# yl602019618/Reconstruction-of-PDE-without-Time-Label

Measured on AMD Instinct MI355X. Metric: snapshot-bags/sec (train step) + rel-L2 drift error, 2D FPE 128² @1/2/4/8 GPU, higher is better.
Workload: dtype f32; 1 GPU; 2d_FPE train_fno.py NIOFP2D_FNO(2,3,100,25,3,12,32,2) (C), grid 128x128; per_gpu_batch=4, global_batch=4, T=100, bag_size=L=randint(50,T) with replacement, dataset_bags=4096, parallelism=dp1, optimizer=Adam lr 0.0005 (fused flat), launch=hip-graph per bag size L (all kernels replayed each step)

## Files before the change

include/blindno.h:

```cpp
#ifndef BLINDNO_H
#define BLINDNO_H

#include <stdint.h>

#ifdef __cplusplus
extern "C" {
#endif

typedef void* blindno_stream_t;

int blindno_abi_version(void);
const char* blindno_error_string(int code);


int blindno_lift_fwd(const float* in, const float* w0, const float* b0, float* x0,
                     int Bn, int N1, int N2, int Cin, int C, int P1, int P2,
                     blindno_stream_t stream);

int blindno_lift_bwd(const float* dx0, const float* in, const float* w0, float* d_in,
                     float* partial, int nchunk,
                     int Bn, int N1, int N2, int Cin, int C, int P1, int P2,
                     blindno_stream_t stream);
int blindno_lift_bwd_nchunk(int Bn, int N1, int N2);

// ... 212 lines not shown
                        int width, blindno_stream_t stream);
int blindno_bagattn_bwd(const float* grid, const float* u, const float* dy, const float* w,
                        const float* A, const float* cs, float* partial, float* dm, float* M,
                        float* du, float* dgt, int B, int L, int S, int width,
                        blindno_stream_t stream);


int blindno_mse(const float* p, const float* t, float* partial, float* grad, int64_t n,
                int nblk, const float* gscale, blindno_stream_t stream);
int blindno_mse_finish(const float* partial, int nblk, int64_t n, float* loss,
                       blindno_stream_t stream);
int blindno_mse_finish_acc(const float* partial, int nblk, int64_t n, float* loss, float* acc,
                           blindno_stream_t stream);
int blindno_mse_fwd(const float* p, const float* t, float* partial, int64_t n, int nblk,
                    float* loss, float* acc, unsigned* counter, float* grad,
                    blindno_stream_t stream);

int blindno_rowsq(const float* a, const float* b, double* out, int rows, int n, int stride,
                  int off_a, int off_b, int den_all, blindno_stream_t stream);

int blindno_gather_flat(const void* const* srcs, const int64_t* offs, const int64_t* ns, int nseg,
                        float* dst, blindno_stream_t stream);
int blindno_gather_batch(const void* const* srcs, void* const* dsts, const int64_t* rows,
                         const int64_t* nsrc, int nseg, const int64_t* ids, int B,
                         blindno_stream_t stream);
int blindno_adam(float* p, const float* g, float* m, float* v, int64_t n, double beta1,
                 double beta2, float eps, float step_size, float bc2s, float gscale,
                 blindno_stream_t stream);


int blindno_gpe_solve(const double* psi0, const double* V, const double* g, const double* kappa,
                      double dx, double dt, int nsteps, int order, int rec_every, double* rec_abs,
                      double* rec_psi, double* psi_out, int B, int Nx, int psi0_batched,
                      blindno_stream_t stream);

int blindno_trapz_rows(const double* a, const double* b, const double* x, double* out, int rows,
                       int n, blindno_stream_t stream);

int blindno_fp_propagate(const double* p0, const double* coef, double* out, int B, int nx,
                         int ny, int nout, int substeps, int degree, double dt_out,
                         blindno_stream_t stream);

int blindno_lift_fwd_g(const float* in, const float* w0, const float* b0, float* x0, int G,
                       int64_t wgs, int Bn, int N1, int N2, int Cin, int C, int P1, int P2,
                       blindno_stream_t stream);
int blindno_lift_bwd_g(const float* dx0, const float* in, const float* w0, float* d_in,
                       float* partial, int nchunk, int G, int64_t wgs, int Bn, int N1, int N2,
                       int Cin, int C, int P1, int P2, blindno_stream_t stream);
int blindno_lift_bag_ok(int G, int Bn, int N1, int N2, int Cin, int C, int P1, int P2);
int blindno_lift_fwd_bag_g(const float* in, const float* w0, const float* b0, float* x0, int G,
                           int64_t wgs, int Bn, int N1, int N2, int Cin, int C, int P1, int P2,
                           const float* ubar, const float* grid, const float* bw, const float* bb,
                           float invL, blindno_stream_t stream);
int blindno_lift_bwd_bag_mix_g(const float* dx0, const float* in, const float* w0, float* d_in,
                               float* partial, int nchunk, int G, int64_t wgs, int Bn, int N1,
                               int N2, int Cin, int C, int P1, int P2, const float* Xs,
                               const float* Gs, float* dWt, float* mpartial, int mnsplit, int K1,
                               int m2, const float* ubar, const float* grid, const float* bw,
                               const float* bb, float invL, float invLb, blindno_stream_t stream);
int blindno_lift_bwd_mix_g(const float* dx0, const float* in, const float* w0, float* d_in,
                           float* partial, int nchunk, int G, int64_t wgs, int Bn, int N1, int N2,
                           int Cin, int C, int P1, int P2, const float* Xs, const float* Gs,
                           float* dWt, float* mpartial, int mnsplit, int K1, int m2,
                           blindno_stream_t stream);
int blindno_project_fwd_g(const float* z, const float* w1, const float* b1, const float* w2,
                          const float* b2, float* out, int G, int64_t wgs, int Bn, int C, int P1,
                          int P2, int Ho, int Wo, int Hd, int Cout, int ostride, int ooff,
                          blindno_stream_t stream);
int blindno_project_bwd_g(const float* z, const float* w1, const float* b1, const float* w2,
                          const float* dout, float* dz, float* partial, int nchunk, int G,
                          int64_t wgs, int Bn, int C, int P1, int P2, int Ho, int Wo, int Hd,
                          int Cout, int ostride, int ooff, blindno_stream_t stream);
int blindno_colpass_g(const float* At, const float* Wt, float* Xs, float* Y, float* Z,
                      const float* FB, const float* GB, int G, int64_t wtgs, int Bn, int Ci,
                      int Co, int P1, int m1, int m2, int P2, int dir, blindno_stream_t stream);
int blindno_mix_wgrad_g(const float* X, const float* Gs, float* dWt, float* partial, int nsplit,
                        int G, int Bn, int Ci, int Co, int K1, int m2, blindno_stream_t stream);
int blindno_rowidft_epi_g(const float* Z, const float* x, const float* wc, const float* bc,
                          float* z, const float* tb, int G, int64_t wgs, int Bn, int C, int P1,
                          int P2, int m2, int act, blindno_stream_t stream);
int blindno_rowidft_bwd_g(const float* Gs, const float* dz, const float* wc, const float* xsrc,
                          float* dx, const float* tb, int G, int64_t wgs, int Bn, int C, int P1,
                          int P2, int m2, int act, blindno_stream_t stream);
int blindno_conv_wgrad_g(const float* dz, const float* x, float* partial, int nchunk, int G,
                         int Bn, int C, int P1, int P2, int act, blindno_stream_t stream);
int blindno_rowdft_wgrad_ok(int Bn, int C, int P1, int P2, int m2);
int blindno_rowdft_wgrad_g(const float* dz, const float* src, float* At, const float* Tp,
                           float* cpartial, int cnchunk, int act, const float* Xs,
                           const float* Gs, float* dWt, float* mpartial, int mnsplit, int K1,
                           int G, int Bn, int C, int P1, int P2, int m2, blindno_stream_t stream);

int blindno_bn_act_nslices(int N, int C, int HW);
int blindno_bn_act_fwd(const float* z, const float* gamma, const float* beta, float* run_mean,
                       float* run_var, float* y, float* save, float* partial, int N, int Npad,
                       int C, int HW, float eps, float momentum, float slope, int training,
                       blindno_stream_t stream);
int blindno_bn_act_bwd(const float* dy, const float* z, const float* gamma, const float* save,
                       float* dz, float* dgamma, float* dbeta, float* partial, float* coef, int N,
                       int Npad, int C, int HW, float slope, int training, blindno_stream_t stream);

int blindno_conv2d_fwd(const float* x, const float* w, const float* b, float* y, int N, int Ci,
                       int Hi, int Wi, int Co, int KH, int KW, int sh, int sw, int ph, int pw,
                       blindno_stream_t stream);
int blindno_conv2d_bwd_data(const float* dy, const float* w, float* dx, int N, int Ci, int Hi,
                            int Wi, int Co, int KH, int KW, int sh, int sw, int ph, int pw,
                            blindno_stream_t stream);
int blindno_conv2d_wgrad_nsplit(int N, int Ci, int Hi, int Wi, int Co, int KH, int KW, int sh,
                                int sw, int ph, int pw);
int blindno_conv2d_bwd_weight(const float* dy, const float* x, float* dwb, float* partial,
                              int nsplit, int N, int Ci, int Hi, int Wi, int Co, int KH, int KW,
                              int sh, int sw, int ph, int pw, blindno_stream_t stream);
int blindno_conv2d_fwd_nsplit(int N, int Ci, int Hi, int Wi, int Co, int KH, int KW, int sh,
                              int sw, int ph, int pw);
int blindno_conv2d_bwd_data_nsplit(int N, int Ci, int Hi, int Wi, int Co, int KH, int KW, int sh,
                                   int sw, int ph, int pw);
int blindno_conv2d_wscratch_floats(int mode, int N, int Ci, int Hi, int Wi, int Co, int KH, int KW,
                                   int sh, int sw, int ph, int pw);
int blindno_conv2d_fwd_split(const float* x, const float* w, const float* b, float* y,
                             float* partial, int nsplit, float* wscratch, int N, int Ci, int Hi,
                             int Wi, int Co, int KH, int KW, int sh, int sw, int ph, int pw,
                             blindno_stream_t stream);
int blindno_conv2d_bwd_data_split(const float* dy, const float* w, float* dx, float* partial,
                                  int nsplit, float* wscratch, int N, int Ci, int Hi, int Wi,
                                  int Co, int KH, int KW, int sh, int sw, int ph, int pw,
                                  blindno_stream_t stream);

int64_t blindno_spectral2d_tables_bytes(int P1, int P2, int m1, int m2);
int blindno_spectral2d_tables_init(void* tables, int P1, int P2, int m1, int m2);
int64_t blindno_spectral_conv2d_workspace_bytes(int Bn, int Ci, int Co, int P1, int P2, int m1,
                                                int m2, int bwd);
int64_t blindno_spectral_conv2d_saved_bytes(int Bn, int Ci, int P1, int m1, int m2);
int blindno_spectral_conv2d_fwd(const float* x, const float* w1, const float* w2, float* y,
                                float* saved, void* work, const void* tables, int Bn, int Ci,
                                int Co, int P1, int P2, int m1, int m2, blindno_stream_t stream);
int blindno_spectral_conv2d_bwd(const float* dy, const float* saved, const float* w1,
                                const float* w2, float* dx, float* dw1, float* dw2, void* work,
                                const void* tables, int Bn, int Ci, int Co, int P1, int P2,
                                int m1, int m2, blindno_stream_t stream);
int64_t blindno_spectral1d_tables_bytes(int P2, int m);
int blindno_spectral1d_tables_init(void* tables, int P2, int m);
int64_t blindno_spectral_conv1d_workspace_bytes(int Bn, int Ci, int Co, int P2, int m, int bwd);
int64_t blindno_spectral_conv1d_saved_bytes(int Bn, int Ci, int m);
int blindno_spectral_conv1d_fwd(const float* x, const float* w, float* y, float* saved,
                                void* work, const void* tables, int Bn, int Ci, int Co, int P2,
                                int m, blindno_stream_t stream);
int blindno_spectral_conv1d_bwd(const float* dy, const float* saved, const float* w, float* dx,
                                float* dw, void* work, const void* tables, int Bn, int Ci,
                                int Co, int P2, int m, blindno_stream_t stream);

int blindno_dwconv_fwd(const float* x, const float* w, const float* b, float* y, int N, int C,
                       int H, int W, int KH, int KW, blindno_stream_t stream);
int blindno_dwconv_bwd_data(const float* dy, const float* w, float* dx, int N, int C, int H,
                            int W, int KH, int KW, blindno_stream_t stream);
int blindno_dwconv_wgrad_nsplit(int N, int C, int H, int W);
int blindno_dwconv_bwd_weight(const float* dy, const float* x, float* dwb, float* partial,
                              int nsplit, int N, int C, int H, int W, int KH, int KW,
                              blindno_stream_t stream);
int blindno_cnx_pw_fwd(const float* xd, const float* sc, const float* lw, const float* lb,
                       const float* w1, const float* b1, const float* w2, const float* b2, float* y,
                       int N, int C, int HW, blindno_stream_t stream);
int blindno_cnx_pw_bwd_nblk(int N, int C, int HW);
int blindno_cnx_pw_bwd(const float* dy, const float* xd, const float* lw, const float* lb,
                       const float* w1, const float* b1, const float* w2, float* dxd,
                       float* dparams, float* partial, int nblk, int N, int C, int HW,
                       blindno_stream_t stream);
int blindno_maxpool_fwd(const float* x, float* y, uint8_t* arg, int NC, int H, int W, int KH,
// ... 66 lines not shown
```

reconstruction-of-pde-without-time-label_amd/blindno/_lib.py:

```python
from __future__ import annotations

import ctypes
import os
import threading

import torch

_HERE = os.path.dirname(os.path.abspath(__file__))
LIB_PATH = os.environ.get("BLINDNO_LIB", os.path.join(_HERE, "libblindno.so"))

SIGNATURES = {
    "blindno_abi_version": "",
    "blindno_lift_fwd": "ppppiiiiiiis",
    "blindno_lift_bwd": "pppppiiiiiiiis",
    "blindno_project_fwd": "ppppppiiiiiiiiiis",
    "blindno_project_bwd": "pppppppiiiiiiiiiiiis",
    "blindno_rowdft": "pppiiiiiis",
    "blindno_rowdft_crop": "pppiiiiiiiis",
    "blindno_rowdft_bag_lift": "ppppppiiiiiiiiis",
    "blindno_rowdft_bag_lift_dg": "pppppppiiiiiiiiis",
    "blindno_rowidft_epi_lift": "ppppppppppiiiiiiiiis",
    "blindno_rowidft_bwd_lift": "ppppppppppiiiiiiiiis",
    "blindno_colpass": "pppppppiiiiiiiis",
    "blindno_colspec_ok": "iiiiii",
    "blindno_colspec_nchunk": "ii",
    "blindno_colspec_bwd_nchunk": "ii",
    "blindno_rowdft_cd": "ppppiiiiiiiis",
    "blindno_rowdft_bag_lift_cd": "pppppiiiiiiiis",
    "blindno_rowdft_bag_lift_cd_pack": "pppppiiiiiiiippppis",
    "blindno_colmix": "pipppiiiiiiiippps",
    "blindno_rowidft_epi_zc": "ppppppppp" + "iiiiiiiiii" + "s",
    "blindno_rowidft_epi_lift_zc": "ppppppppppppp" + "iiiiiiiiiii" + "s",
    "blindno_rowidft_bwd_zc": "pppppppppp" + "iiiiiiiii" + "s",
    "blindno_rowidft_bwd_lift_zc": "ppppppppppp" + "iiiiiiiiii" + "s",
    "blindno_rowidft_bwd_lift_zc_mix": "ppppppppppp" + "iiiiiiiiii" + "ppppi" + "s",
    "blindno_rowdft_cd_bag": "pppi" + "ppp" + "iiiiiii" + "s",
    "blindno_rowidft_bwd_zc_bag": "pppp" + "i" + "pppppppp" + "iiiiiiiii" + "s",
    "blindno_mix_wgrad": "ppppiiiiiis",
    "blindno_mix_wgrad_part": "pppiiiiiiis",
    "blindno_mix_wgrad_multi": "ppppis",
    "blindno_mix_wgrad_multi_u": "ppppppis",
    "blindno_mix1d": "ppppiiiiiis",
    "blindno_rowidft_epi": "ppppppiiiiiis",
    "blindno_rowidft_epi_crop": "pppppp" + "iiiiiiii" + "s",
    "blindno_rowidft_bwd": "pppppppiiiiiis",
    "blindno_rowidft_bwd_crop": "pppppppiiiiiiiis",
    "blindno_rowidft_bwd_rd": "pppppppiiiiiiiipps",
    "blindno_rowidft_epi_rd": "ppppppiiiiiippis",
    "blindno_rowidft_epi_lift_rd": "ppppppppppiiiiiiiiippis",
    "blindno_conv_wgrad": "pppiiiiiis",
    "blindno_reduce_partials": "ppiis",
    "blindno_spectrum_tile_layout": "iiiii",
    "blindno_pack_w2d": "pppiiiiis",
    "blindno_unpack_w2d": "pppiiiiis",
    "blindno_pack_w1d": "ppiiiis",
    "blindno_bagmean_fwd": "pppppiiiiis",
    "blindno_bagmean_bwd": "pppiiiiis",
    "blindno_mse": "pppplips",
    "blindno_mse_finish": "pilps",
    "blindno_mse_finish_acc": "pilpps",
    "blindno_mse_fwd": "ppplipppps",
    "blindno_rowsq": "pppiiiiiis",
    "blindno_adam": "pppplddffffs",
    "blindno_gpe_solve": "ppppddiiipppiiis",
    "blindno_trapz_rows": "ppppiis",
    "blindno_lift_bwd_nchunk": "iii",
    "blindno_conv_wgrad_nchunk": "iii",
    "blindno_rowidft_bwd_nchunk": "iiiii",
    "blindno_set_rowfuse": "i",
    "blindno_set_colfuse": "i",
    "blindno_project_bwd_nchunk": "iii",
    "blindno_project_bwd_nchunk_heads": "iii",
    "blindno_mix_wgrad_nsplit": "iiiii",
    "blindno_lift_fwd_g": "ppppiliiiiiiis",
    "blindno_lift_fwd_bag_g": "ppppiliiiiiiippppfs",
    "blindno_lift_bag_ok": "iiiiiiii",
    "blindno_lift_bwd_g": "pppppiiliiiiiiis",
    "blindno_lift_bwd_mix_g": "pppppiiliiiiiiippppiiis",
    "blindno_lift_bwd_bag_mix_g": "pppppiiliiiiiiippppiiippppffs",
    "blindno_project_fwd_g": "ppppppiliiiiiiiiiis",
    "blindno_project_bwd_g": "pppppppiiliiiiiiiiiis",
    "blindno_colpass_g": "pppppppiliiiiiiiis",
    "blindno_mix_wgrad_g": "ppppiiiiiiis",
    "blindno_rowidft_epi_g": "ppppppiliiiiiis",
    "blindno_rowidft_bwd_g": "ppppppiliiiiiis",
    "blindno_conv_wgrad_g": "pppiiiiiiis",
    "blindno_rowdft_wgrad_ok": "iiiii",
    "blindno_rowdft_wgrad_g": "pppppiippppiiiiiiiis",
    "blindno_bagmean_fwd_w": "pppppp" + "iiiii" + "s",
    "blindno_project_bwd_w": "pppppppp" + "i" + "iiiiiiiiiii" + "s",
    "blindno_project_bag_stats_floats": "iii",
    "blindno_project_bag_bwd_nchunk": "iii",
    "blindno_project_bag_fwd": "ppppppppp" + "iiiiiiii" + "s",
    "blindno_project_bag_bwd": "ppppppp" + "i" + "iiiiiiii" + "s",
    "blindno_pack_w2d_2": "ppppp" + "iiiii" + "s",
    "blindno_unpack_w2d_2": "ppppp" + "iiiii" + "s",
    "blindno_bn_act_nslices": "iii",
    "blindno_bn_act_fwd": "ppppppppiiiifffis",
    "blindno_bn_act_bwd": "pppppppppiiiifis",
    "blindno_gather_flat": "pppips",
    "blindno_gather_batch": "ppppipis",
    "blindno_reduce_partials_multi": "ppppis",
    "blindno_reduce_partials_pieces": "ppppppis",
    "blindno_reduce_partials_pieces_u": "pppppppppis",
    "blindno_reduce_segs_limit": "i",
    "blindno_finish_multi": "pppppppppippppis",
    "blindno_unpack_w2d_multi": "ppppis",
    "blindno_pack_w2d_multi": "ppppis",
    "blindno_fp_propagate": "pppiiiiiids",
    "blindno_bagattn_nchunk": "i",
    "blindno_bagattn_fwd": "pppppppp" + "iiii" + "s",
    "blindno_bagattn_bwd": "ppppppppppp" + "iiii" + "s",
    "blindno_conv2d_fwd": "pppp" + "iiiiiiiiiii" + "s",
    "blindno_conv2d_bwd_data": "ppp" + "iiiiiiiiiii" + "s",
    "blindno_conv2d_wgrad_nsplit": "iiiiiiiiiii",
    "blindno_conv2d_bwd_weight": "pppp" + "i" + "iiiiiiiiiii" + "s",
    "blindno_conv2d_fwd_nsplit": "iiiiiiiiiii",
    "blindno_conv2d_fwd_split": "ppppp" + "i" + "p" + "iiiiiiiiiii" + "s",
    "blindno_conv2d_bwd_data_nsplit": "iiiiiiiiiii",
    "blindno_conv2d_bwd_data_split": "pppp" + "i" + "p" + "iiiiiiiiiii" + "s",
    "blindno_conv2d_wscratch_floats": "i" + "iiiiiiiiiii",
    "blindno_spectral2d_tables_bytes": "iiii",
    "blindno_spectral2d_tables_init": "piiii",
    "blindno_spectral_conv2d_workspace_bytes": "iiiiiiii",
    "blindno_spectral_conv2d_saved_bytes": "iiiii",
    "blindno_spectral_conv2d_fwd": "ppppppp" + "iiiiiii" + "s",
    "blindno_spectral_conv2d_bwd": "ppppppppp" + "iiiiiii" + "s",
    "blindno_spectral1d_tables_bytes": "ii",
    "blindno_spectral1d_tables_init": "pii",
    "blindno_spectral_conv1d_workspace_bytes": "iiiiii",
    "blindno_spectral_conv1d_saved_bytes": "iii",
    "blindno_spectral_conv1d_fwd": "pppppp" + "iiiii" + "s",
    "blindno_spectral_conv1d_bwd": "ppppppp" + "iiiii" + "s",
    "blindno_dwconv_fwd": "pppp" + "iiiiii" + "s",
    "blindno_dwconv_bwd_data": "ppp" + "iiiiii" + "s",
    "blindno_dwconv_wgrad_nsplit": "iiii",
    "blindno_dwconv_bwd_weight": "pppp" + "i" + "iiiiii" + "s",
    "blindno_cnx_pw_fwd": "ppppppppp" + "iii" + "s",
    "blindno_cnx_pw_bwd_nblk": "iii",
    "blindno_cnx_pw_bwd": "pppppppppp" + "iiii" + "s",
    "blindno_maxpool_fwd": "ppp" + "iiiii" + "s",
    "blindno_maxpool_bwd": "ppp" + "iiiii" + "s",
    "blindno_convt_fwd": "pppp" + "iiiiiiiii" + "s",
    "blindno_convt_bwd_data": "ppp" + "iiiiiiiii" + "s",
    "blindno_convt_wgrad_nparts": "iii",
    "blindno_convt_bwd_weight": "pppp" + "iiiiiiiii" + "s",
    "blindno_tok_gram_nchunk": "l",
    "blindno_tok_attn_save_floats": "iil",
    "blindno_tok_attn_fwd": "ppppppp" + "iil" + "f" + "s",
    "blindno_tok_attn_bwd_scratch_floats": "ii",
    "blindno_tok_attn_bwd": "pppppppp" + "iil" + "s",
    "blindno_deeponet_bag_nblk": "i",
    "blindno_deeponet_bag_fwd": "pppppp" + "iiii" + "f" + "s",
    "blindno_deeponet_bag_bwd": "pppppppp" + "iiiii" + "f" + "s",
    "blindno_spectral3d_ok": "iiiiiiiii",
    "blindno_colpass3d": "ppppppp" + "iiiiiiiiii" + "s",
    "blindno_pack_w3d": "ppppp" + "iiiiiiii" + "s",
    "blindno_unpack_w3d": "ppppp" + "iiiiiiii" + "s",
    "blindno_lift3d_fwd": "pppp" + "iiiiiiiii" + "s",
    "blindno_lift3d_bwd_nchunk": "iiii",
    "blindno_lift3d_bwd": "ppppp" + "i" + "iiiiiiiii" + "s",
    "blindno_project3d_fwd": "pppppp" + "iiiiiiiiii" + "s",
    "blindno_project3d_bwd_nchunk": "iiii",
    "blindno_project3d_bwd": "ppppppp" + "i" + "iiiiiiiiii" + "s",
}

SIGNATURES_CONV3D = {
    "blindno_conv3d_fwd_nsplit": "i" * 15,
# ... 120 lines not shown
```

reconstruction-of-pde-without-time-label_amd/blindno/ops.py:

```python
from __future__ import annotations

import contextlib
import ctypes
import math
from typing import List, Optional, Sequence, Tuple

import torch

from ._lib import BlindnoError, call, ptr, query, stream_ptr

F32 = torch.float32

MIX_F16 = False

BAG_STATS = True
BAG_STATS_MAX_BYTES = 4 << 30

COLSPEC = True
HEAD_BWD_MERGED = True
UNPACK_FOLD = True
HOST_ENC_MIX = True
HOST_PACK = True


# ... 1154 lines not shown
        offs.append(o)
        o += t.numel()
    return offs, o


def pack_heads_ahead(meta: FNOMeta, shape, prms, device):
    if not (GROUPED_HEADS and grouped_ok(meta, shape, prms)):
        return
    G, n = len(prms), meta.n_layers
    P1 = _fno_geometry(shape, meta)[4]
    K1 = kept_rows_count(meta.m1, P1)
    C = meta.width
    Wt_all = torch.empty(n, G, meta.m2, K1, C, C, 2, dtype=F32, device=device)
    segs = [(prms[g][2 + 4 * k], prms[g][3 + 4 * k]) for k in range(n) for g in range(G)]
    pack_ahead(segs, [Wt_all[k, g] for k in range(n) for g in range(G)], P1, Wt_all)


def grouped_ok(meta: FNOMeta, inp, prms) -> bool:
    if meta.dim != 2 or len(prms) != 2:
        return False
    n = meta.n_layers
    fc1w, fc2w = prms[0][2 + 4 * n], prms[0][4 + 4 * n]
    Hd, Cout = fc1w.shape[0], fc2w.shape[0]
    if Hd != 128 or meta.width > 15 or Cout > 2:
        return False
    if any(a.shape != b.shape for a, b in zip(prms[0], prms[1])):
        return False
    Bg, N1, N2, Cin, P1, P2, Ho, Wo = _fno_geometry(inp, meta)
    return (Bg * Ho * Wo) % 64 == 0 and P1 % 4 == 0


def _sub(buf, off):
    return buf[off:] if off else buf


class _GroupWeights:

    def __init__(self, smalls):
        d = None
        direct = all(t.is_contiguous() and t.dtype == F32 for sm in smalls for t in sm)
        for g in range(1, len(smalls)):
            for a, b in zip(smalls[0], smalls[g]):
                diff = b.data_ptr() - a.data_ptr()
                if diff % (4 * g) or (d is not None and diff != g * d):
                    direct = False
                    break
                d = diff // g
        if direct and d:
            self.base, self.buf, self.S = list(smalls[0]), None, d // 4
        else:
            self.offs, self.S = _offsets(smalls[0])
            self.buf = torch.cat([t.reshape(-1) for sm in smalls for t in sm])
            self.base = None

    def p(self, i):
        return ptr(self.base[i]) if self.base is not None else ptr(_sub(self.buf, self.offs[i]))


def fno_forward_grouped(meta: FNOMeta, inp, prms, bag=None):
    G = len(prms)
    Bg, N1, N2, Cin, P1, P2, Ho, Wo = _fno_geometry(inp if bag is None else bag.shape(inp), meta)
    Bn = G * Bg
    C, n = meta.width, meta.n_layers
    smalls = [_small_params(p, n, 2) for p in prms]
    small = _GroupWeights(smalls)
    S = small.S
    x0 = _empty(Bn, C, P1, P2, like=inp)
    if bag is None:
        call("blindno_lift_fwd_g", ptr(inp), small.p(0), small.p(1), ptr(x0),
             G, S, Bn, N1, N2, Cin, C, P1, P2, stream_ptr())
    else:
        call("blindno_lift_fwd_bag_g", None, small.p(0), small.p(1), ptr(x0), G, S, Bn, N1, N2, Cin, C,
             P1, P2, ptr(inp), ptr(bag.grid), ptr(bag.w), ptr(bag.b), 1.0, stream_ptr())
    K1 = kept_rows_count(meta.m1, P1)
    K1p = 16 * ((K1 + 15) // 16)
    FB, GB = twiddle_cols(P1, meta.m1, inp.device)
    src, act = x0, 0
    Xs, Wts, zs = [], [], []
    segs = [(prms[g][2 + 4 * k], prms[g][3 + 4 * k]) for k in range(n) for g in range(G)]
    Wt_all = take_packed(segs, P1)
    if Wt_all is None:
        Wt_all = _empty(n, G, meta.m2, K1, C, C, 2, like=inp)
        _pack_into(segs, [Wt_all[k, g] for k in range(n) for g in range(G)], P1)
    for k in range(n):
        Wt = Wt_all[k]
        At = k_rowdft(src, Bn, C, P1, P2, meta.m2, act)
        X = _empty(Bn, meta.m2, C, K1, 2, like=inp)
        Y = _empty(Bn, meta.m2, C, K1p, 2, like=inp)
        Z = _empty(Bn, P1, meta.m2, C, 2, like=inp)
        call("blindno_colpass_g", ptr(At), ptr(Wt), ptr(X), ptr(Y), ptr(Z), ptr(FB), ptr(GB), G,
             Wt[0].numel(), Bn, C, C, P1, meta.m1, meta.m2, P2, _mixdir(0), stream_ptr())
        z = _empty(Bn, C, P1, P2, like=inp)
        call("blindno_rowidft_epi_g", ptr(Z), ptr(src), small.p(2 + 2 * k),
             small.p(3 + 2 * k), ptr(z), ptr(twiddle_rowinv(P2, meta.m2, inp.device)),
             G, S, Bn, C, P1, P2, meta.m2, act, stream_ptr())
        Xs.append(X)
        Wts.append(Wt)
        zs.append(z)
        src, act = z, 1
    o1 = 2 + 2 * n
    Hd, Cout = smalls[0][o1].shape[0], smalls[0][o1 + 2].shape[0]
    out = _empty(Bg, Ho, Wo, G * Cout, like=inp)
    call("blindno_project_fwd_g", ptr(zs[-1]), small.p(o1), small.p(o1 + 1),
         small.p(o1 + 2), small.p(o1 + 3), ptr(out), G, S, Bn, C, P1, P2,
         Ho, Wo, Hd, Cout, G * Cout, 0, stream_ptr())
    return out, (small, x0, Xs, Wts, zs)


_DZ_PAD = {}


def _padded_grad_buffer(shape, device):
    key = (tuple(shape), str(device))
    t = _DZ_PAD.get(key)
    if t is None:
        t = torch.zeros(shape, dtype=F32, device=device)
        if not torch.cuda.is_current_stream_capturing():
            _DZ_PAD[key] = t
    return t


def fno_backward_grouped(meta: FNOMeta, inp, prms, saved, gout, need_inp_grad, bag=None):
    G = len(prms)
    Bg, N1, N2, Cin, P1, P2, Ho, Wo = _fno_geometry(inp if bag is None else bag.shape(inp), meta)
    Bn = G * Bg
    C, n = meta.width, meta.n_layers
    small, x0, Xs, Wts, zs = saved
    smalls = [_small_params(p, n, 2) for p in prms]
    S = small.S
    o1 = 2 + 2 * n
    Hd, Cout = smalls[0][o1].shape[0], smalls[0][o1 + 2].shape[0]
    gout = _c(gout)
    grads = [[None] * len(p) for p in prms]
    off_fc1 = 2 + 4 * n
    dz = _padded_grad_buffer((Bn, C, P1, P2), inp.device)
    np_p = Hd * C + Hd + Cout * Hd + Cout
    nchunk = query("blindno_project_bwd_nchunk_heads", Bg, Ho, Wo)
    partial = _empty(nchunk, G, np_p, like=inp)
    call("blindno_project_bwd_g", ptr(zs[-1]), small.p(o1), small.p(o1 + 1),
         small.p(o1 + 2), ptr(gout), ptr(dz), ptr(partial), nchunk, G, S, Bn, C, P1, P2,
         Ho, Wo, Hd, Cout, G * Cout, 0, stream_ptr())
    gp = reduce_partials(partial, nchunk, G * np_p).view(G, np_p)
    for g in range(G):
        o = 0
        grads[g][off_fc1] = gp[g, o:o + Hd * C].view(Hd, C); o += Hd * C
        grads[g][off_fc1 + 1] = gp[g, o:o + Hd]; o += Hd
        grads[g][off_fc1 + 2] = gp[g, o:o + Cout * Hd].view(Cout, Hd); o += Cout * Hd
        grads[g][off_fc1 + 3] = gp[g, o:o + Cout]
    K1 = kept_rows_count(meta.m1, P1)
    K1p = 16 * ((K1 + 15) // 16)
    FB, GB = twiddle_cols(P1, meta.m1, inp.device)
    tb = twiddle_rowinv(P2, meta.m2, inp.device)
    np_c = C * C + C
    ns = query("blindno_mix_wgrad_nsplit", Bg, C, C, K1, meta.m2)
    nch = query("blindno_conv_wgrad_nchunk", Bg, P1, P2)
    merged = HEAD_BWD_MERGED and query("blindno_rowdft_wgrad_ok", Bn, C, P1, P2, meta.m2) == 1
    pending = None

    def mix_buffers():
        dWt = _empty(G, meta.m2, K1, C, C, 2, like=inp)
        part = _empty(ns, G, meta.m2 * K1 * C * C * 2, like=inp) if ns > 1 else None
        return dWt, part

    def mix_grads(kk, dWt):
        o = 2 + 4 * kk
        if _DEFER is not None:
            dws = [d for g in range(G) for d in unpack_w2d(dWt[g], prms[g][o], P1)]
        else:
            dws = [torch.empty_like(prms[g][o]) for g in range(G) for _ in range(2)]
            call("blindno_unpack_w2d_2", ptr(dWt), ptr(dws[0]), ptr(dws[1]), ptr(dws[2]), ptr(dws[3]), C,
                 C, meta.m1, meta.m2, P1, stream_ptr())
        for g in range(G):
            grads[g][o], grads[g][o + 1] = dws[2 * g], dws[2 * g + 1]

    defer_mix = _DEFER is not None and not merged

    def mix_launch(kk, Xk, Gk):
        dWt, part = mix_buffers()
        if defer_mix:
            _DEFER.mix.append((Xk, Gk, part if ns > 1 else dWt, (Bn, C, C, K1, meta.m2, ns, G)))
            if ns > 1:
                _DEFER.red.append([part, dWt, ns, dWt.numel(), []])
        else:
            call("blindno_mix_wgrad_g", ptr(Xk), ptr(Gk), ptr(dWt), ptr(part) if part is not None else None,
                 ns, G, Bn, C, C, K1, meta.m2, stream_ptr())
        mix_grads(kk, dWt)

    for k in reversed(range(n)):
        off = 2 + 4 * k
        src, act = (x0, 0) if k == 0 else (zs[k - 1], 1)
        Wt = Wts[k]
        pc = _empty(nch, G, np_c, like=inp)
        if merged:
            At = _empty(Bn, meta.m2, C, P1, 2, like=inp)
            mx = (None, None, None, None)
            if pending is not None:
                dWt, part = mix_buffers()
                mx = (pending[1], pending[2], dWt, part)
            call("blindno_rowdft_wgrad_g", ptr(dz), ptr(src), ptr(At), ptr(twiddle_mfma(P2, meta.m2, inp.device)),
                 ptr(pc), nch, act, *[ptr(t) if t is not None else None for t in mx], ns, K1, G, Bn, C,
                 P1, P2, meta.m2, stream_ptr())
            if pending is not None:
                mix_grads(pending[0], dWt)
        else:
            At = k_rowdft(dz, Bn, C, P1, P2, meta.m2, 0)
        Gs = _empty(Bn, meta.m2, C, K1, 2, like=inp)
        Y = _empty(Bn, meta.m2, C, K1p, 2, like=inp)
        GZ = _empty(Bn, P1, meta.m2, C, 2, like=inp)
        call("blindno_colpass_g", ptr(At), ptr(Wt), ptr(Gs), ptr(Y), ptr(GZ), ptr(FB), ptr(GB), G,
             Wt[0].numel(), Bn, C, C, P1, meta.m1, meta.m2, P2, _mixdir(1), stream_ptr())
        if merged and not defer_mix:
            pending = (k, Xs[k], Gs)
        else:
            mix_launch(k, Xs[k], Gs)
            if not merged:
                call("blindno_conv_wgrad_g", ptr(dz), ptr(src), ptr(pc), nch, G, Bn, C, P1, P2, act,
                     stream_ptr())
        gc = reduce_partials(pc, nch, G * np_c).view(G, np_c)
        for g in range(G):
            grads[g][off + 2] = gc[g, :C * C].view_as(prms[g][off + 2])
            grads[g][off + 3] = gc[g, C * C:]
        dz_new = _empty(Bn, C, P1, P2, like=inp)
        call("blindno_rowidft_bwd_g", ptr(GZ), ptr(dz), small.p(2 + 2 * k), ptr(src),
             ptr(dz_new), ptr(tb), G, S, Bn, C, P1, P2, meta.m2, act, stream_ptr())
        dz = dz_new
    np_l = C * Cin + C
    nchunk = query("blindno_lift_bwd_nchunk", Bg, N1, N2)
    partial = _empty(nchunk, G, np_l, like=inp)
    d_inp = torch.empty_like(inp) if need_inp_grad else None
    mx = (None, None, None, None)
    if pending is not None:
        dWt, part = mix_buffers()
        mx = (pending[1], pending[2], dWt, part)
    if bag is None:
        call("blindno_lift_bwd_mix_g", ptr(dz), ptr(inp), small.p(0), ptr(d_inp), ptr(partial), nchunk, G,
             S, Bn, N1, N2, Cin, C, P1, P2, *[ptr(t) if t is not None else None for t in mx], ns, K1,
             meta.m2, stream_ptr())
    else:
        if d_inp is None:
            d_inp = torch.empty_like(inp)
        call("blindno_lift_bwd_bag_mix_g", ptr(dz), None, small.p(0), ptr(d_inp), ptr(partial), nchunk,
             G, S, Bn, N1, N2, Cin, C, P1, P2, *[ptr(t) if t is not None else None for t in mx], ns,
             K1, meta.m2, ptr(inp), ptr(bag.grid), ptr(bag.w), ptr(bag.b), 1.0, 1.0, stream_ptr())
    if pending is not None:
        mix_grads(pending[0], dWt)
    gl = reduce_partials(partial, nchunk, G * np_l).view(G, np_l)
    for g in range(G):
        grads[g][0] = gl[g, :C * Cin].view(C, Cin)
        grads[g][1] = gl[g, C * Cin:]
    return d_inp, grads


GROUPED_HEADS = True


class HeadPairFn(torch.autograd.Function):

    @staticmethod
    def forward(ctx, meta0, meta1, n0, side, h, *prm):
        bag = None
        if isinstance(meta0, tuple):
            meta0, bag = meta0
        require_device(h, *prm)
        h = _c(h)
        prm = [_c(p) for p in prm]
        p0, p1 = prm[:n0], prm[n0:]
        hin = h if bag is None else bag.shape(h)
        ctx.grouped = GROUPED_HEADS and meta0.__dict__ == meta1.__dict__ and grouped_ok(meta0, hin, [p0, p1])
        ctx.bag = bag
        if bag is not None and not ctx.grouped:
            raise BlindnoError("HeadPairFn: a bag-mean input needs the grouped heads")
        if ctx.grouped:
            out, saved = fno_forward_grouped(meta0, h, [p0, p1], bag=bag)
            ctx.save_for_backward(h, *prm)
            ctx.meta = (meta0, meta1, n0, side, None)
            ctx.s0, ctx.s1 = saved, None
            return out
        main = torch.cuda.current_stream(h.device)
        side.wait_stream(main)
        o0, s0 = fno_forward(meta0, h, p0, save=True)
        with torch.cuda.stream(side):
            o1, s1 = fno_forward(meta1, h, p1, save=True)
        main.wait_stream(side)
        h.record_stream(side)
        o1.record_stream(main)
        out = torch.cat([o0, o1], dim=-1)
        ctx.save_for_backward(h, *prm)
        ctx.meta = (meta0, meta1, n0, side, o0.shape[-1])
        ctx.s0, ctx.s1 = s0, s1
        return out

    @staticmethod
    def backward(ctx, gout):
        meta0, meta1, n0, side, c0 = ctx.meta
        t = ctx.saved_tensors
        h, prm = t[0], list(t[1:])
        p0, p1 = prm[:n0], prm[n0:]
        need = ctx.needs_input_grad[4]
        gout = _c(gout)
        if ctx.grouped:
            dh, gr = fno_backward_grouped(meta0, h, [p0, p1], ctx.s0, gout, need, bag=ctx.bag)
            ctx.s0 = ctx.bag = None
            grads = [g if ctx.needs_input_grad[5 + i] else None for i, g in enumerate(gr[0] + gr[1])]
            return (None, None, None, None, dh, *grads)
        g0 = gout[..., :c0].contiguous()
        g1 = gout[..., c0:].contiguous()
        main = torch.cuda.current_stream(h.device)
        side.wait_stream(main)
        with torch.cuda.stream(side):
            d1, gr1 = fno_backward(meta1, h, p1, ctx.s1, g1, need)
        d0, gr0 = fno_backward(meta0, h, p0, ctx.s0, g0, need)
        main.wait_stream(side)
        g1.record_stream(side)
        for g in ([d1] if d1 is not None else []) + [g for g in gr1 if g is not None]:
            g.record_stream(main)
        ctx.s0 = ctx.s1 = None
        dh = d0 + d1 if need else None
        grads = [g if ctx.needs_input_grad[5 + i] else None for i, g in enumerate(gr0 + gr1)]
        return (None, None, None, None, dh, *grads)




def k_rowdft_bag_lift(X, idx_t, w0, b0, Dg, B, T, L, N1, N2, C, P1, P2, m2):
    At = _empty(B * L, m2, C, P1, 2, like=X)
    call("blindno_rowdft_bag_lift_dg", ptr(X), ptr(idx_t), ptr(w0), ptr(b0), ptr(Dg), ptr(At),
         ptr(twiddle_mfma(P2, m2, X.device)), B, T, L, N1, N2, C, P1, P2, m2, stream_ptr())
    return At


_DG_CACHE = {}


def _grid_planes(grid, N1, N2, P1, P2, m2):
    key = (grid.device, grid.data_ptr(), grid._version, N1, N2, P1, P2, m2)
    capturing = torch.cuda.is_current_stream_capturing()
# ... 742 lines not shown
```

Baseline: 3665 snapshot-bags/s.

## Fuse inverse row DFT epilogue with next layer's forward row DFT

Adds a kernel that computes the inverse row DFT plus pointwise conv epilogue for a Fourier layer, then applies GELU and immediately computes the next layer's forward row DFT from LDS. The head forward loop uses it for every layer except the last. This removes one full read of the activation and one kernel launch per layer. It also writes a GELU'd copy (fz) for the next epilogue's residual input, which adds an extra write and more LDS use that may lower occupancy.

```diff
diff --git a/include/blindno.h b/include/blindno.h
--- a/include/blindno.h
+++ b/include/blindno.h
@@ -318,6 +318,11 @@
 int blindno_rowidft_bwd_g(const float* Gs, const float* dz, const float* wc, const float* xsrc,
                           float* dx, const float* tb, int G, int64_t wgs, int Bn, int C, int P1,
                           int P2, int m2, int act, blindno_stream_t stream);
+int blindno_rowidft_epi_chain_ok(int Bn, int C, int P1, int P2, int m2);
+int blindno_rowidft_epi_chain_g(const float* Z, const float* x, const float* wc, const float* bc,
+                                float* z, const float* tb, int G, int64_t wgs, int Bn, int C,
+                                int P1, int P2, int m2, int act, float* At, const float* Tp,
+                                int act_next, float* fz, blindno_stream_t stream);
 int blindno_conv_wgrad_g(const float* dz, const float* x, float* partial, int nchunk, int G,
                          int Bn, int C, int P1, int P2, int act, blindno_stream_t stream);
 int blindno_rowdft_wgrad_ok(int Bn, int C, int P1, int P2, int m2);
diff --git a/reconstruction-of-pde-without-time-label_amd/blindno/_lib.py b/reconstruction-of-pde-without-time-label_amd/blindno/_lib.py
--- a/reconstruction-of-pde-without-time-label_amd/blindno/_lib.py
+++ b/reconstruction-of-pde-without-time-label_amd/blindno/_lib.py
@@ -84,6 +84,8 @@
     "blindno_mix_wgrad_g": "ppppiiiiiiis",
     "blindno_rowidft_epi_g": "ppppppiliiiiiis",
     "blindno_rowidft_bwd_g": "ppppppiliiiiiis",
+    "blindno_rowidft_epi_chain_ok": "iiiii",
+    "blindno_rowidft_epi_chain_g": "pppppp" + "il" + "iiiiii" + "pp" + "i" + "p" + "s",
     "blindno_conv_wgrad_g": "pppiiiiiiis",
     "blindno_rowdft_wgrad_ok": "iiiii",
     "blindno_rowdft_wgrad_g": "pppppiippppiiiiiiiis",
diff --git a/reconstruction-of-pde-without-time-label_amd/blindno/ops.py b/reconstruction-of-pde-without-time-label_amd/blindno/ops.py
--- a/reconstruction-of-pde-without-time-label_amd/blindno/ops.py
+++ b/reconstruction-of-pde-without-time-label_amd/blindno/ops.py
@@ -1260,18 +1260,33 @@
     if Wt_all is None:
         Wt_all = _empty(n, G, meta.m2, K1, C, C, 2, like=inp)
         _pack_into(segs, [Wt_all[k, g] for k in range(n) for g in range(G)], P1)
+    chain = (HEADS_CHAIN and not MIX_F16 and K1p <= 64 and
+             query("blindno_rowidft_epi_chain_ok", Bn, C, P1, P2, meta.m2) == 1)
+    At_next = None
+    xin, xact = src, act
     for k in range(n):
         Wt = Wt_all[k]
-        At = k_rowdft(src, Bn, C, P1, P2, meta.m2, act)
+        At = At_next if At_next is not None else k_rowdft(src, Bn, C, P1, P2, meta.m2, act)
+        At_next = None
         X = _empty(Bn, meta.m2, C, K1, 2, like=inp)
         Y = _empty(Bn, meta.m2, C, K1p, 2, like=inp)
         Z = _empty(Bn, P1, meta.m2, C, 2, like=inp)
         call("blindno_colpass_g", ptr(At), ptr(Wt), ptr(X), ptr(Y), ptr(Z), ptr(FB), ptr(GB), G,
              Wt[0].numel(), Bn, C, C, P1, meta.m1, meta.m2, P2, _mixdir(0), stream_ptr())
         z = _empty(Bn, C, P1, P2, like=inp)
-        call("blindno_rowidft_epi_g", ptr(Z), ptr(src), small.p(2 + 2 * k),
-             small.p(3 + 2 * k), ptr(z), ptr(twiddle_rowinv(P2, meta.m2, inp.device)),
-             G, S, Bn, C, P1, P2, meta.m2, act, stream_ptr())
+        if chain and k + 1 < n:
+            At_next = _empty(Bn, meta.m2, C, P1, 2, like=inp)
+            fz = _empty(Bn, C, P1, P2, like=inp)
+            call("blindno_rowidft_epi_chain_g", ptr(Z), ptr(xin), small.p(2 + 2 * k),
+                 small.p(3 + 2 * k), ptr(z), ptr(twiddle_rowinv(P2, meta.m2, inp.device)),
+                 G, S, Bn, C, P1, P2, meta.m2, xact, ptr(At_next),
+                 ptr(twiddle_mfma(P2, meta.m2, inp.device)), 1, ptr(fz), stream_ptr())
+            xin, xact = fz, 0
+        else:
+            call("blindno_rowidft_epi_g", ptr(Z), ptr(xin), small.p(2 + 2 * k),
+                 small.p(3 + 2 * k), ptr(z), ptr(twiddle_rowinv(P2, meta.m2, inp.device)),
+                 G, S, Bn, C, P1, P2, meta.m2, xact, stream_ptr())
+            xin, xact = z, 1
         Xs.append(X)
         Wts.append(Wt)
         zs.append(z)
@@ -1430,6 +1445,7 @@
 
 
 GROUPED_HEADS = True
+HEADS_CHAIN = True
 
 
 class HeadPairFn(torch.autograd.Function):
diff --git a/reconstruction-of-pde-without-time-label_amd/csrc/rowchain.hip b/reconstruction-of-pde-without-time-label_amd/csrc/rowchain.hip
--- /dev/null
+++ b/reconstruction-of-pde-without-time-label_amd/csrc/rowchain.hip
@@ -0,0 +1,202 @@
+#include "common.h"
+#include "blindno.h"
+#include "gelu_pk.h"
+#include "kernels.h"
+
+using namespace blindno;
+
+namespace {
+
+typedef float f32x4 __attribute__((ext_vector_type(4)));
+
+constexpr int kChainWaves = 10;
+
+__device__ __forceinline__ f32x4 gelu4(f32x4 x) {
+  using namespace blindno::gelu_pk;
+  const f32x2 v[2] = {{x[0], x[1]}, {x[2], x[3]}};
+  const f32x2 hk[2] = {v[0] * splat2(kK), v[1] * splat2(kK)};
+  f32x2 cdf[2];
+  norm_cdf_pairs<2>(hk, cdf);
+  const f32x2 g0 = v[0] * cdf[0], g1 = v[1] * cdf[1];
+  return (f32x4){g0.x, g0.y, g1.x, g1.y};
+}
+
+template <int CM, int KSM>
+__global__ __launch_bounds__(64 * kChainWaves) void rowchain_wide_kernel(
+    const float* __restrict__ Z, const float* __restrict__ xs, const float* __restrict__ wc,
+    const float* __restrict__ bc, float* __restrict__ out, const float* __restrict__ TB,
+    float* __restrict__ At, const float* __restrict__ Tp, float* __restrict__ fz, int Bn, int P1,
+    int P2, int m2, int Npad, int act, int act_next, int Bg, int64_t wgs) {
+  constexpr int C = CM;
+  constexpr int NGM = CM / 4;
+  extern __shared__ __attribute__((aligned(16))) float lds[];
+  const int KS = m2 >> 1;
+  const int NT = P2 >> 4;
+  const int NNT = Npad >> 4;
+  const int HB = P1 >> 4;
+  const int HW = P1 * P2;
+  f32x4* sZ = reinterpret_cast<f32x4*>(lds);
+  f32x4* sF = sZ + KS * 64;
+  f32x4* sT = sF + 4 * NT * 64;
+  const int lane = threadIdx.x & 63;
+  const int wave = uniform_int(threadIdx.x >> 6);
+  const int nwaves = (int)blockDim.x >> 6;
+  const int c16 = lane & 15, g = lane >> 4;
+  const int cg = (int)blockIdx.x % NGM;
+  const int blk = (int)blockIdx.x / NGM;
+  const int n = blk / HB, h0 = (blk - n * HB) << 4;
+  const int h = h0 + c16;
+  const bool has_wc = wc != nullptr;
+  const f32x4 zero4 = {0.f, 0.f, 0.f, 0.f};
+
+  __shared__ __attribute__((aligned(16))) float sw[4 * CM + 4];
+  if (has_wc) {
+    const int64_t goff = wgs ? (int64_t)(n / Bg) * wgs : 0;
+    for (int e = threadIdx.x; e < 4 * CM + 4; e += blockDim.x)
+      sw[e] = e < 4 * CM ? wc[goff + 4 * cg * C + e] : bc[goff + 4 * cg + e - 4 * CM];
+  }
+  {
+    const int q0 = (n * P1 + h0) >> 2;
+    for (int e = threadIdx.x; e < KS * 64; e += blockDim.x) {
+      const int s = e >> 6, l = e & 63;
+      const int q = q0 + ((l & 15) >> 2);
+      sZ[e] = *reinterpret_cast<const f32x4*>(
+          Z + (unsigned)(((q * NGM + cg) * KS + s) * 64 + 16 * (l >> 4) + 4 * (l & 3)));
+    }
+  }
+  for (int e = threadIdx.x; e < NT * 4 * Npad; e += blockDim.x)
+    sT[e] = reinterpret_cast<const f32x4*>(Tp)[e];
+
+  const unsigned fbase = (unsigned)(n * C * HW + h * P2);
+  float av[KSM];
+  f32x4 xin[CM];
+  auto load_ops = [&](int t) {
+    const unsigned off = fbase + (unsigned)(16 * t + 4 * g);
+#pragma unroll
+    for (int s = 0; s < KSM; ++s) av[s] = s < KS ? TB[(unsigned)((s * NT + t) * 64 + lane)] : 0.f;
+    if (has_wc) {
+#pragma unroll
+      for (int i = 0; i < CM; ++i) xin[i] = *reinterpret_cast<const f32x4*>(xs + off + (unsigned)(i * HW));
+    }
+  };
+  if (wave < NT) load_ops(wave);
+  __syncthreads();
+
+  for (int t = wave; t < NT; t += nwaves) {
+    asm volatile("" ::: "memory");
+    const unsigned off = fbase + (unsigned)(16 * t + 4 * g);
+    if (t != wave) load_ops(t);
+    if (has_wc && act) {
+#pragma unroll
+      for (int i = 0; i < CM; ++i) xin[i] = gelu4(xin[i]);
+    }
+    f32x4 d[4];
+#pragma unroll
+    for (int c = 0; c < 4; ++c) d[c] = zero4;
+#pragma unroll
+    for (int s = 0; s < KSM; ++s)
+      if (s < KS) {
+        const f32x4 zb = sZ[s * 64 + lane];
+#pragma unroll
+        for (int c = 0; c < 4; ++c)
+          d[c] = __builtin_amdgcn_mfma_f32_16x16x4f32(av[s], zb[c], d[c], 0, 0, 0);
+      }
+#pragma unroll
+    for (int c = 0; c < 4; ++c) {
+      f32x4 y = d[c];
+      if (has_wc) {
+#pragma unroll
+        for (int r = 0; r < 4; ++r) y[r] += sw[4 * CM + c];
+#pragma unroll
+        for (int i = 0; i < CM; i += 4) {
+          const f32x4 wv = *reinterpret_cast<const f32x4*>(sw + c * CM + i);
+#pragma unroll
+          for (int r = 0; r < 4; ++r) {
+            float v = y[r];
+            v = fmaf(wv[0], xin[i][r], v);
+            v = fmaf(wv[1], xin[i + 1][r], v);
+            v = fmaf(wv[2], xin[i + 2][r], v);
+            v = fmaf(wv[3], xin[i + 3][r], v);
+            y[r] = v;
+          }
+        }
+      }
+      *reinterpret_cast<f32x4*>(out + off + (unsigned)((4 * cg + c) * HW)) = y;
+      const f32x4 fy = act_next ? gelu4(y) : y;
+      sF[(c * NT + t) * 64 + lane] = fy;
+      if (fz) *reinterpret_cast<f32x4*>(fz + off + (unsigned)((4 * cg + c) * HW)) = fy;
+    }
+  }
+  __syncthreads();
+
+  for (int it = wave; it < 4 * NNT; it += nwaves) {
+    const int c = it & 3, nt = it >> 2;
+    const f32x4* tp = sT + g * Npad + 16 * nt + c16;
+    const f32x4* sf = sF + c * NT * 64 + lane;
+    f32x4 acc = zero4, acc1 = zero4;
+    for (int t = 0; t < NT; t += 2) {
+      const f32x4 tb = tp[t * 4 * Npad];
+      const f32x4 ya = sf[t * 64];
+      const bool two = t + 1 < NT;
+      const f32x4 tb1 = two ? tp[(t + 1) * 4 * Npad] : zero4;
+      const f32x4 ya1 = two ? sf[(t + 1) * 64] : zero4;
+#pragma unroll
+      for (int s = 0; s < 4; ++s) {
+        acc = __builtin_amdgcn_mfma_f32_16x16x4f32(tb[s], ya[s], acc, 0, 0, 0);
+        acc1 = __builtin_amdgcn_mfma_f32_16x16x4f32(tb1[s], ya1[s], acc1, 0, 0, 0);
+      }
+    }
+    acc += acc1;
+#pragma unroll
+    for (int rp = 0; rp < 2; ++rp) {
+      const int k = 8 * nt + 2 * g + rp;
+      if (k < m2)
+        *reinterpret_cast<float2*>(At + ((((int64_t)n * m2 + k) * C + 4 * cg + c) * P1 + h) * 2) =
+            make_float2(acc[2 * rp], acc[2 * rp + 1]);
+    }
+  }
+}
+
+bool aligned16(const void* p) { return ((uintptr_t)p & 15) == 0; }
+
+}
+
+BLINDNO_API int blindno_rowidft_epi_chain_ok(int Bn, int C, int P1, int P2, int m2) {
+  if (!rowinv_tile_layout(Bn, C, P1, P2, m2)) return 0;
+  if (!(C == 12 || C == 16) || m2 / 2 > 16 || (P1 & 15) || (P2 & 15) || P2 > 256 ||
+      m2 > P2 / 2 + 1)
+    return 0;
+  if ((int64_t)Bn * (P1 / 16) * (C / 4) >= INT32_MAX) return 0;
+  return 1;
+}
+
+BLINDNO_API int blindno_rowidft_epi_chain_g(const float* Z, const float* x, const float* wc,
+                                            const float* bc, float* z, const float* tb, int G,
+                                            int64_t wgs, int Bn, int C, int P1, int P2, int m2,
+                                            int act, float* At, const float* Tp, int act_next,
+                                            float* fz, void* stream) {
+  if (!Z || !z || !tb || !At || !Tp || G < 1 || Bn < 1 || Bn % G) return (int)hipErrorInvalidValue;
+  if (!blindno_rowidft_epi_chain_ok(Bn, C, P1, P2, m2)) return (int)hipErrorInvalidValue;
+  if (wc && (!x || !bc)) return (int)hipErrorInvalidValue;
+  if (!aligned16(Z) || !aligned16(x) || !aligned16(z) || !aligned16(Tp) || !aligned16(fz))
+    return (int)hipErrorInvalidValue;
+  const int Bg = Bn / G;
+  if (G == 1) wgs = 0;
+  const int Npad = ((2 * m2 + 15) / 16) * 16;
+  const int ks = m2 / 2, NT = P2 / 16;
+  const unsigned nb = (unsigned)(Bn * (P1 / 16) * (C / 4));
+  const int nw = NT < 4 ? 4 : (NT < kChainWaves ? NT : kChainWaves);
+  const size_t sh = sizeof(float) * 4 * (64 * ((size_t)ks + 4 * (size_t)NT) + (size_t)NT * 4 * Npad);
+  if (sh > 160 * 1024) return (int)hipErrorInvalidValue;
+  hipStream_t st = (hipStream_t)stream;
+#define RC(CM_, KS_)                                                                          \
+  rowchain_wide_kernel<CM_, KS_><<<nb, 64 * nw, sh, st>>>(Z, x, wc, bc, z, tb, At, Tp, fz, Bn, \
+                                                          P1, P2, m2, Npad, act, act_next, Bg, wgs)
+  if (C == 12) {
+    if (ks <= 8) RC(12, 8); else RC(12, 16);
+  } else {
+    if (ks <= 8) RC(16, 8); else RC(16, 16);
+  }
+#undef RC
+  return (int)hipGetLastError();
+}
```

Result: no change. 3700 snapshot-bags/s (median of 6 runs) (+0.9%).
